# 0Setsuna0/SoftbodyUnity

Hardware: AMD Instinct MI355X
Metric: particle-substeps/sec (higher is better)
Workload: dtype f32

## Files before the change

softbodyunity_amd/csrc/kernel_types.hpp:

```cpp
#pragma once
#include <hip/hip_runtime.h>
#include <stdint.h>

#include "stream_codec.hpp"

namespace sbk {

struct TickParams {
    float h, inv_h, hgx, hgy, hgz, kd, at_d, at_v, at_b;
    float pnx, pny, pnz, pd;
    int32_t plane_on;
    float pad[2];
};

constexpr int kKindFirst = 0, kKindMid = 1, kKindLast = 2, kKindLayer = 3, kKindPeek = 4, kKindMidKinematic = 5;
constexpr bool kind_is_kinematic(int k) { return k == kKindMidKinematic; }
constexpr int kind_base(int k) { return kind_is_kinematic(k) ? kKindMid : k; }
constexpr bool kind_has_mark(int k) { return k != kKindLayer; }
constexpr bool kind_rounds_before_mark(int k) { return k != kKindFirst; }
constexpr bool kind_rounds_after_mark(int k) { return k == kKindFirst || kind_base(k) == kKindMid; }
constexpr bool kind_ends_tick(int k) { return k == kKindLast || k == kKindPeek; }
constexpr bool kind_reads_prev(int k) { return kind_base(k) == kKindMid || k == kKindLast; }
constexpr bool kind_touches_prev(int k) { return k == kKindFirst || kind_reads_prev(k); }
constexpr bool kind_writes_peek(int k) { return k == kKindPeek; }
constexpr bool kind_may_read_ghosts(int k) { return k == kKindMid || k == kKindLast; }
constexpr bool kind_gathers(int k) { return k == kKindLayer; }

struct TileDesc {
    int32_t n_local, run_count, n_rounds;
    int32_t gather_begin;
    uint32_t s_begin;
    uint32_t s_hdr;
    uint32_t s_len;
    uint32_t packed_lanes;
    int32_t run_overflow;
    int32_t n_pal;
    int32_t n_steps;
    uint32_t s_items;
    int2 runs[10];
};
constexpr int kInlineRuns = 10;
constexpr int kWide8MaxTiles = 768;
#ifndef SB_REG_ROUNDS
#define SB_REG_ROUNDS 4
#endif
#ifndef SB_REG_ROUNDS_NARROW
#define SB_REG_ROUNDS_NARROW 3
#endif
constexpr int kRegRoundsWide = SB_REG_ROUNDS, kRegRoundsNarrow = SB_REG_ROUNDS_NARROW;
#ifdef SB_REG_COMPACT_ONLY
constexpr bool kRegFullSlots = false;
#else
constexpr bool kRegFullSlots = true;
#endif
constexpr bool kLanePackDecodable = kRegRoundsNarrow >= kLanePackRounds;
constexpr int kMaxRoundsLds = 128;

typedef float f32x3_t __attribute__((ext_vector_type(3)));
struct PosView {
    float *xyz;
    const float *w;
};

constexpr int kMaxMassPalette = 64;

struct TileArgs {
    PosView pos;
    const uint8_t *w8;
    const float *wpal;
    float *prev;
    float *vel;
    const TileDesc *tiles;
    const int2 *runs_overflow;
    const uint32_t *stream;
    const TickParams *tp;
    const int32_t *gather;
    int32_t max_local;
    int32_t rounds_dwords;
    int32_t pal_dwords;
    int32_t win_dwords;
    int32_t tile_base;
    int32_t w_uniform;
    int32_t item_waves;
    int32_t store_through;
    union {
        const float *ghost_src;
        uint2 *prev_code;
    };
    int32_t n_owned;
    float *peek_out;
    const int32_t *kin_map;
    float *kin_target;
};
constexpr int kHaloNone = 0, kHaloGhosts = 1;

constexpr int kNarrowTileThreads = 128;
constexpr int kQuadTileThreads = 512;
constexpr int kWideTileThreads = 256;
constexpr int kRoundSlots = 256;
constexpr int kSmallTile = 512, kLargeTile = 1024;
typedef float f32x3 __attribute__((ext_vector_type(3)));

typedef float f32x4 __attribute__((ext_vector_type(4)));
typedef uint32_t u32x4 __attribute__((ext_vector_type(4)));

constexpr int kMaxPeers = 8;
struct PeerSlot {
    int32_t n_send, n_recv;
    int32_t send_off[kMaxPeers + 1];
// ... 25 lines not shown
```

softbodyunity_amd/csrc/launch_shape.hpp:

```cpp
#pragma once
#include "kernel_types.hpp"
#include "tables_host.hpp"

namespace sbt {

struct LaunchShape { int threads, ppt; bool quads; };
inline bool same_width(const LaunchShape &a, const LaunchShape &b) { return a.threads == b.threads && a.ppt == b.ppt; }

constexpr LaunchShape kShapeNarrow{sbk::kNarrowTileThreads, sbk::kSmallTile / sbk::kNarrowTileThreads, false};
constexpr LaunchShape kShapeWide{sbk::kWideTileThreads, sbk::kSmallTile / sbk::kWideTileThreads, false};
constexpr LaunchShape kShapeWideLarge{sbk::kWideTileThreads, sbk::kLargeTile / sbk::kWideTileThreads, false};
constexpr LaunchShape kShapeEight{sbk::kQuadTileThreads, sbk::kSmallTile / sbk::kQuadTileThreads, false};
constexpr LaunchShape kShapeEightLarge{sbk::kQuadTileThreads, sbk::kLargeTile / sbk::kQuadTileThreads, false};

inline LaunchShape tile_launch_shape(const TilingScalars &D, int tile_lanes, int quad_lanes, int narrow_min_tiles, int n_tiles_in_launch, bool ghosts) {
    const bool small = D.max_local <= sbk::kSmallTile;
    const bool narrow = small && (D.packed_lanes ? D.packed_lanes == sbk::kLanePackLanes : (tile_lanes ? tile_lanes == sbk::kNarrowTileThreads : n_tiles_in_launch >= narrow_min_tiles));
    const bool quad8 = D.has_quads && quad_lanes == sbk::kQuadTileThreads;
    const bool wide8 = small && !D.has_quads && !D.packed_lanes && (tile_lanes ? tile_lanes == sbk::kQuadTileThreads : n_tiles_in_launch <= sbk::kWide8MaxTiles);
    const bool quads = ghosts ? false : D.has_quads;
    LaunchShape sh = quads && quad8 ? (small ? kShapeEight : kShapeEightLarge) : wide8 ? kShapeEight : narrow ? kShapeNarrow : small ? kShapeWide : kShapeWideLarge;
    sh.quads = quads;
    return sh;
}

inline bool tiling_always_narrow(const TilingScalars &D, int tile_lanes) {
    if (D.n_tiles == 0) return true;
    return D.max_local <= sbk::kSmallTile && !D.has_quads && (D.packed_lanes ? D.packed_lanes == sbk::kLanePackLanes : tile_lanes == sbk::kNarrowTileThreads);
}
constexpr int64_t kPrevCodeMaxParticles = (int64_t)1 << 26;
struct PrevCodeInputs {
    int world = 1;
    int halo_slots = 0;
    int tile_lanes = 0;
    bool w_palette = false;
    int steps_between_tiles = 0;
    int64_t n_local = 0;
};
inline bool use_prev_codes(const TilingScalars &T0, const TilingScalars &T1, const PrevCodeInputs &in) {
    if (in.world != 1 || in.halo_slots != 0) return false;
    if (!in.w_palette) return false;
    if (in.steps_between_tiles != 0) return false;
    if (T0.n_tiles == 0 || in.n_local > kPrevCodeMaxParticles) return false;
    return tiling_always_narrow(T0, in.tile_lanes) && tiling_always_narrow(T1, in.tile_lanes);
}

}
```

softbodyunity_amd/csrc/schedule.hip:

```cpp
#include "solver_internal.hpp"
#include "launch_shape.hpp"
#include "tile_kernel.hip.hpp"
#include "aux_kernels.hip.hpp"

namespace sbi {

sbk::TickParams tick_params(const sb_solver *s, float dt, int substeps) {
    sbk::TickParams t{};
    volatile float S = (float)substeps;
    volatile float h = dt / S;
    t.h = h;
    volatile float inv_h = 1.0f / h;
    t.inv_h = inv_h;
    volatile float hx = h * s->desc.gravity[0], hy = h * s->desc.gravity[1], hz = h * s->desc.gravity[2];
    t.hgx = hx; t.hgy = hy; t.hgz = hz;
    volatile float td = s->desc.damping * h;
    volatile float kd = 1.0f - td;
    t.kd = kd < 0.0f ? 0.0f : (float)kd;
    volatile float h2 = h * h;
    volatile float ad = s->mesh->kind[0].compliance / h2;
    volatile float av = s->mesh->kind[1].compliance / h2;
    volatile float av36 = 36.0f * av;
    volatile float ab = s->mesh->kind[2].compliance / h2;
    t.at_d = ad; t.at_v = av36; t.at_b = ab;
// ... 108 lines not shown

void halo_exchange_calls(sb_solver *s, int slot, hipStream_t st) {
    if (!halo_slot_active(s, slot) || s->peer.enabled) return;
    DevHalo &D = *s->halos[slot];
    const size_t fl = sbt::ghost_floats((size_t)slot);
    for (size_t k = 0; k < D.peers.size(); ++k) {
        int cs = D.send_off[k + 1] - D.send_off[k], cr = D.recv_off[k + 1] - D.recv_off[k];
        if (s->loopback) cs = cr = std::min(cs, cr);
        if (cs) NCCL_CHECK(rccl().Send(s->d_sendbuf.p + fl * D.send_off[k], fl * (size_t)cs, ncclFloat, s->loopback ? 0 : D.peers[k], s->comm, st));
        if (cr) NCCL_CHECK(rccl().Recv(s->d_recvbuf.p + fl * D.recv_off[k], fl * (size_t)cr, ncclFloat, s->loopback ? 0 : D.peers[k], s->comm, st));
    }
}

void halo_exchange_post(sb_solver *s, int slot, hipStream_t st) {
    if (!halo_slot_active(s, slot) || s->peer.enabled) return;
    launch_halo_unpack(s, *s->halos[slot], slot, st);
}

void ExchangeTimer::mark(hipStream_t st, bool join) {
    Event e;
    if (free_list.empty()) e.create(); else { e = std::move(free_list.back()); free_list.pop_back(); }
    HIP_CHECK(hipEventRecord(e, st));
    (join ? join_pending : pending).push_back(std::move(e));
}
void ExchangeTimer::recycle() {
    for (auto *v : {&pending, &join_pending}) {
        free_list.insert(free_list.end(), std::make_move_iterator(v->begin()), std::make_move_iterator(v->end()));
        v->clear();
    }
}

void halo_exchange(sb_solver *s, int slot, hipStream_t st) {
    if (!st) st = s->stream;
    if (!halo_slot_active(s, slot)) return;
    const bool timed = s->xtimer.enabled && !s->capturing;
    if (timed) s->xtimer.mark(st);
    if (!s->peer.enabled) halo_exchange_pre(s, slot, st);
    if (timed) s->xtimer.mark(st);
    if (s->peer.enabled) halo_exchange_pre(s, slot, st);
    if (!s->peer.enabled) {
        NCCL_CHECK(rccl().GroupStart());
        try {
            halo_exchange_calls(s, slot, st);
        } catch (...) {
            (void)rccl().GroupEnd();
            throw;
        }
        NCCL_CHECK(rccl().GroupEnd());
    }
    halo_exchange_post(s, slot, st);
    if (timed) s->xtimer.mark(st);
}

template <int KIND, bool Q, int THREADS, int PPT, bool W, int G, bool C = false>
void launch_tile_kernel(const sb_solver *s, const DevTiling &D, const sbk::TileDesc *tiles_at_base, int n_wg, const sbk::TileArgs &A) {
    hipLaunchKernelGGL((sbk::tile_kernel<KIND, Q, THREADS, PPT, W, G, C>), dim3(n_wg), dim3(THREADS), D.lds_bytes + s->lds_pad, s->stream, tiles_at_base, n_wg, A);
}
template <int KIND, bool Q, bool W, int G>
void launch_tile_shaped(const sb_solver *s, const DevTiling &D, const sbt::LaunchShape &sh, const sbk::TileDesc *tiles_at_base, int n_wg, const sbk::TileArgs &A) {
    using namespace sbt;
    if (same_width(sh, kShapeEight)) return launch_tile_kernel<KIND, Q, kShapeEight.threads, kShapeEight.ppt, W, G>(s, D, tiles_at_base, n_wg, A);
    if constexpr (Q) if (same_width(sh, kShapeEightLarge)) return launch_tile_kernel<KIND, Q, kShapeEightLarge.threads, kShapeEightLarge.ppt, W, G>(s, D, tiles_at_base, n_wg, A);
    if (same_width(sh, kShapeNarrow)) return launch_tile_kernel<KIND, Q, kShapeNarrow.threads, kShapeNarrow.ppt, W, G>(s, D, tiles_at_base, n_wg, A);
    if (same_width(sh, kShapeWide)) return launch_tile_kernel<KIND, Q, kShapeWide.threads, kShapeWide.ppt, W, G>(s, D, tiles_at_base, n_wg, A);
    if (same_width(sh, kShapeWideLarge)) return launch_tile_kernel<KIND, Q, kShapeWideLarge.threads, kShapeWideLarge.ppt, W, G>(s, D, tiles_at_base, n_wg, A);
    throw std::runtime_error("internal: no tile kernel is built for the launch shape asked for");
}

template <int KIND>
void launch_tile(sb_solver *s, DevTiling &D, int tile_begin = 0, int tile_end = -1, int halo = sbk::kHaloNone, const sbk::TileDesc *table = nullptr) {
    const bool ghosts = halo == sbk::kHaloGhosts;
    if (tile_end < 0) tile_end = D.n_tiles;
    if (tile_end <= tile_begin) return;
    sbk::TileArgs A{};
    A.pos = s->pos_view(); A.w8 = s->d_w8.p; A.wpal = s->d_wpal.p; A.prev = s->d_prev.p; A.vel = s->d_vel.p;
    A.tiles = D.tiles.p; A.runs_overflow = D.runs_overflow.p; A.stream = D.stream.p;
    A.tp = s->d_tp.p;
    A.gather = D.gather.p;
    A.w_uniform = s->w_uniform ? 1 : 0;
    A.item_waves = D.item_waves;
    A.store_through = tile_end - tile_begin <= s->store_through_max_tiles ? 3 : s->store_through_large;
    A.ghost_src = ghosts ? s->d_recvbuf.p : nullptr; A.n_owned = (int32_t)s->n_owned;
    A.peek_out = sbk::kind_writes_peek(KIND) ? s->d_peek.p : nullptr;
    A.kin_map = sbk::kind_is_kinematic(KIND) ? s->d_kin_map.p : nullptr; A.kin_target = sbk::kind_is_kinematic(KIND) ? s->d_kin_target.p : nullptr;
    A.max_local = D.max_local; A.win_dwords = D.win_dwords; A.tile_base = tile_begin; A.pal_dwords = D.pal_dwords; A.rounds_dwords = D.rounds_dwords;
    const sbk::TileDesc *tiles_at_base = table ? table : D.tiles.p + tile_begin;
    const int n_wg = tile_end - tile_begin;
    const sbt::LaunchShape sh = sbt::tile_launch_shape(D, s->tile_lanes, s->quad_lanes, s->narrow_min_tiles, n_wg, ghosts);
    constexpr bool kCanGhost = sbk::kind_may_read_ghosts(KIND);
    if (ghosts && !(kCanGhost && !D.has_quads)) throw std::runtime_error("internal: ghost-reading tile kernel requested for a launch that has none");
    const bool W = s->w_palette;
    if constexpr (sbk::kind_touches_prev(KIND)) if (s->prev_codes) {
        if (ghosts || sh.quads || !W || !sbt::same_width(sh, sbt::kShapeNarrow)) throw std::runtime_error("internal: previous-position codes are on, but the launch is not 128 x 4 spring-only with palette masses");
        A.prev_code = s->d_prev_code.p;
        return launch_tile_kernel<KIND, false, sbt::kShapeNarrow.threads, sbt::kShapeNarrow.ppt, true, sbk::kHaloNone, true>(s, D, tiles_at_base, n_wg, A);
    }
    if (ghosts) {
        if constexpr (kCanGhost) W ? launch_tile_shaped<KIND, false, true, sbk::kHaloGhosts>(s, D, sh, tiles_at_base, n_wg, A) : launch_tile_shaped<KIND, false, false, sbk::kHaloGhosts>(s, D, sh, tiles_at_base, n_wg, A);
    } else if (sh.quads) W ? launch_tile_shaped<KIND, true, true, sbk::kHaloNone>(s, D, sh, tiles_at_base, n_wg, A) : launch_tile_shaped<KIND, true, false, sbk::kHaloNone>(s, D, sh, tiles_at_base, n_wg, A);
    else W ? launch_tile_shaped<KIND, false, true, sbk::kHaloNone>(s, D, sh, tiles_at_base, n_wg, A) : launch_tile_shaped<KIND, false, false, sbk::kHaloNone>(s, D, sh, tiles_at_base, n_wg, A);
}

struct LaunchTimer {
    std::vector<Event> ev;
    std::vector<int> slot;
    hipStream_t stream;
    void begin(int which) {
        Event a, b;
        a.create(); b.create();
        HIP_CHECK(hipEventRecord(a, stream));
        ev.push_back(std::move(a)); ev.push_back(std::move(b)); slot.push_back(which);
    }
    void end() { HIP_CHECK(hipEventRecord(ev.back(), stream)); }
};

void launch_tick_kernel(sb_solver *s, int it, int substeps, LaunchTimer *lt, int tile_begin = 0, int tile_end = -1, bool kin = false) {
    const int tl = s->plan->plan.tiling ? (it & 1) : 0;
    DevTiling &D = s->tiling[tl];
    if (lt && D.n_tiles) lt->begin(it == 0 ? 2 + (int)s->gcolours.size() : (it == substeps ? 3 + (int)s->gcolours.size() : tl));
    const int halo_in = s->fused_unpack && tl == 1 ? sbk::kHaloGhosts : sbk::kHaloNone;
    if (it == 0) launch_tile<sbk::kKindFirst>(s, D, tile_begin, tile_end);
    else if (it < substeps && kin) launch_tile<sbk::kKindMidKinematic>(s, D, tile_begin, tile_end);
    else if (it < substeps) launch_tile<sbk::kKindMid>(s, D, tile_begin, tile_end, halo_in);
    else launch_tile<sbk::kKindLast>(s, D, tile_begin, tile_end, halo_in);
    if (lt && D.n_tiles) lt->end();
}

void launch_t2_layer(sb_solver *s, int layer, LaunchTimer *lt, bool with_halo = true) {
    const auto rg = s->t2_layer_range[layer];
    if (with_halo) halo_exchange(s, 2 + (int)s->gcolours.size() + layer);
    if (rg.second <= rg.first) return;
    if (lt) lt->begin(4 + (int)s->gcolours.size());
    launch_tile<sbk::kKindLayer>(s, s->tiling[2], rg.first, rg.second);
    if (lt) lt->end();
}

void launch_gcolour(sb_solver *s, int gc, LaunchTimer *lt) {
    DevGColour &G = *s->gcolours[gc];
    if (G.count == 0) return;
    if (lt) lt->begin(2 + gc);
    dim3 grid((G.count + 255) / 256);
    if (G.type == 0)
        hipLaunchKernelGGL(sbk::global_distance_kernel, grid, dim3(256), 0, s->stream, s->pos_view(), G.ij.p, G.rest.p, G.count,
                           s->d_tp.p);
    else
        hipLaunchKernelGGL(sbk::global_quad_kernel, grid, dim3(256), 0, s->stream, s->pos_view(), G.quad.p, G.rest2.p, G.count,
                           G.type, s->d_tp.p);
// ... 416 lines not shown
```

softbodyunity_amd/csrc/solver_internal.hpp:

```cpp
#pragma once
#include <hip/hip_runtime.h>
#include <rccl/rccl.h>
#include <dlfcn.h>

#include <algorithm>
#include <array>
#include <atomic>
#include <chrono>
#include <climits>
#include <cmath>
#include <cstdio>
#include <cstdlib>
#include <cstring>
#include <limits>
#include <map>
#include <memory>
#include <mutex>
#include <type_traits>
#include <stdexcept>
#include <string>
#include <utility>
#include <vector>

#include "../../include/softbody.h"
// ... 95 lines not shown
    StepKind kind;
    TileRange range;
    bool kin;
    int it, substeps;
    int index;
};
struct TickShape { int substeps; bool fuse, defer_last, kin; };

struct ExchangeTimer {
    bool enabled = false;
    std::vector<Event> pending, join_pending, free_list;
    void mark(hipStream_t st, bool join = false);
    void recycle();
};

}

using sbi::DevBuf; using sbi::DevGColour; using sbi::DevHalo; using sbi::DevTiling;

struct sb_plan {
    sbp::Plan plan;
    sbp::LocalPlan local;
    bool owns_local = true;
};

struct sb_solver {
    sb_desc desc;
    bool finalized = false;
    sbi::Stream stream;
    sbi::Event ev0, ev1;
    ncclComm_t comm = nullptr;
    bool loopback = false;
    int schedule = SB_SCHEDULE_SERIAL_EAGER;
    uint64_t plan_hash = 0;
    sbi::Stream comm_stream;
    sbi::Event ev_boundary, ev_halo;
    bool overlap_halo = false;
    std::shared_ptr<sbi::AuthoredMesh> mesh = std::make_shared<sbi::AuthoredMesh>();
    bool sharded = false;
    sb_domain domain{};
    std::vector<int32_t> global_id;
    std::unique_ptr<sb_plan> plan;
    int64_t dev_bytes = 0;
    int64_t n_owned = 0, n_local = 0;
    DevBuf<float> d_pos3;
    DevBuf<float> d_wf;
    DevBuf<uint8_t> d_w8;
    DevBuf<float> d_wpal;
    bool w_palette = false;
    bool w_uniform = false;
    sbk::PosView pos_view() const { return sbk::PosView{d_pos3.p, d_wf.p}; }
    DevBuf<float> d_prev, d_vel;
    bool prev_codes = false;
    DevBuf<uint2> d_prev_code;
    DevBuf<sbk::TickParams> d_tp;
    DevBuf<float> d_sendbuf, d_recvbuf;
    DevTiling tiling[3];
    std::vector<std::pair<int32_t, int32_t>> t2_layer_range;
    std::vector<std::unique_ptr<DevGColour>> gcolours;
    std::vector<std::unique_ptr<DevHalo>> halos;
    sbk::TickParams tp_host{};
    bool tp_valid = false;
    sbi::GraphCache graphs;
    bool deferred = false;
    int deferred_substeps = 0;
    uint32_t tune_flags = 0;
    int win_dwords_cap = 0;
    int prev_offset_bytes = 0;
    bool lazy_tick = true;
    int tile_lanes = 0;
    int quad_lanes = 512;
    int store_through_max_tiles = 6144;
    int store_through_large = 0;
    int narrow_min_tiles = 10240;
    size_t lds_pad = 0;
    bool pack_tiles = true;
    bool fused_unpack = false;
    bool graph_rccl = false;
    std::vector<float> h_stage;
    struct AutoSchedule {
        int state = 0;
        int tick = 0;
        sbi::Event ev[8];
        int n[2] = {0, 0};
        double decided_ms[2] = {0, 0};
    } calib;
    bool group_walk = false;
    bool capturing = false;
    sbi::ExchangeTimer xtimer;
    struct PeerState {
        bool enabled = false, linked = false, fine_grained = false;
        uint32_t *mailbox = nullptr;
        size_t bytes = 0, data_off_words = 0, off_table = 0;
        int n_slots = 0;
        std::vector<uint32_t *> remote;
        std::vector<uint8_t> opened;
        std::vector<std::vector<uint32_t>> my_off;
        std::vector<sbk::PeerSlot> slots;
        DevBuf<uint32_t> local;
        sbi::HostBuf<uint32_t> h_error;
        size_t slot_base(int slot, int world) const { return sbt::mailbox_slot_base(slot, world); }
        ~PeerState() {
            for (size_t r = 0; r < remote.size(); ++r) if (opened[r] && remote[r]) (void)hipIpcCloseMemHandle(remote[r]);
            if (mailbox) (void)hipFree(mailbox);
        }
    } peer;
// ... 121 lines not shown
```

softbodyunity_amd/csrc/tables.hip:

```cpp
#include "solver_internal.hpp"
#include "launch_shape.hpp"

namespace sbi {

sbp::Input make_input(const float *rest, int32_t n, const int32_t *d, int64_t md, const int32_t *v, int64_t mv,
                      const int32_t *b, int64_t mb) {
    sbp::Input in;
    in.rest = rest; in.n = n; in.dist_ij = d; in.m_d = md; in.vol = v; in.m_v = mv; in.bend = b; in.m_b = mb;
    return in;
}

sbp::Domain to_domain(const sb_domain &d) {
    sbp::Domain D;
    D.set = true; D.n_global = d.n_global; D.ell = d.spacing; D.fill = d.fill > 0 && d.fill <= 1 ? d.fill : 1.0;
    for (int a = 0; a < 3; ++a) { D.lo[a] = d.lo[a]; D.hi[a] = d.hi[a]; }
    return D;
}
sbp::Opts plan_opts(int rank, int world, const int32_t dims[3], int32_t tile_particles, int32_t partition, uint32_t plan_flags,
                    int64_t m_v, int64_t m_b, const sb_domain *domain) {
    sbp::Opts o;
    if (domain) {
        o.domain = to_domain(*domain);
        if (domain->four_vertex_constraints) m_v += 1;
    }
// ... 71 lines not shown
    opt.peer_enabled = s->peer.enabled; opt.sharded = s->sharded; opt.plan_hash = s->plan_hash;
    opt.plan_shape = opt.peer_enabled && L.world > 1 ? plan_shape(s) : 0u;
    sbt::HostTables H;
    sbt::build_state(in, opt, H);
    s->n_owned = H.n_owned; s->n_local = H.n_local;
    s->w_palette = H.w_palette; s->w_uniform = H.w_uniform;
    s->d_pos3.upload(H.pos3, s->dev_bytes);
    s->d_wf.upload(H.wf, s->dev_bytes);
    if (H.w_palette) s->d_w8.upload(H.w8, s->dev_bytes);
    s->d_wpal.upload(H.wpal, s->dev_bytes);
    s->d_vel.upload(H.vel, s->dev_bytes);
    for (std::vector<float> *v : {&H.pos3, &H.wf, &H.vel}) std::vector<float>().swap(*v);
    std::vector<uint8_t>().swap(H.w8);
    s->d_prev.alloc((size_t)s->n_local * 3, s->dev_bytes, (size_t)s->prev_offset_bytes / sizeof(float));
    HIP_CHECK(hipMemset(s->d_prev.p, 0, (size_t)s->n_local * 3 * sizeof(float)));
    s->d_tp.alloc(1, s->dev_bytes);
    for (int tl = 0; tl < 3; ++tl) {
        sbt::build_tiling(in, opt, tl, H);
        sbt::HostTiling &T = H.T[tl];
        DevTiling &D = s->tiling[tl];
        static_cast<sbt::TilingScalars &>(D) = T;
        D.tiles.upload(T.tiles, s->dev_bytes); D.runs_overflow.upload(T.runs_overflow, s->dev_bytes);
        D.stream.upload(T.stream, s->dev_bytes);
        D.gather.upload(T.gather, s->dev_bytes);
        T.release_arrays();
    }
    s->t2_layer_range = H.t2_layer_range;
    sbt::build_gcolours(in, H);
    for (const sbt::HostGColour &G : H.gcolours) {
        auto D = std::make_unique<DevGColour>();
        D->type = G.type; D->count = G.count;
        if (G.type == 0) { D->ij.upload(G.ij, s->dev_bytes); D->rest.upload(G.rest, s->dev_bytes); }
        else { D->quad.upload(G.quad, s->dev_bytes); D->rest2.upload(G.rest2, s->dev_bytes); }
        s->gcolours.push_back(std::move(D));
    }
    sbt::build_halos(in, opt, H);
    for (sbt::HostHalo &G : H.halos) {
        auto D = std::make_unique<DevHalo>();
        D->send_idx.upload(G.send_idx, s->dev_bytes); D->recv_idx.upload(G.recv_idx, s->dev_bytes);
        D->peers = std::move(G.peers); D->send_off = std::move(G.send_off); D->recv_off = std::move(G.recv_off);
        s->halos.push_back(std::move(D));
    }
    s->d_sendbuf.alloc(H.send_floats, s->dev_bytes);
    s->d_recvbuf.alloc(H.recv_floats, s->dev_bytes);
    if (H.recv_floats) HIP_CHECK(hipMemset(s->d_recvbuf.p, 0, H.recv_floats * sizeof(float)));
    s->fused_unpack = H.fused_unpack;
    if (s->peer.enabled && L.world > 1) alloc_mailbox(s, H.mailbox);
    sbt::PrevCodeInputs pc;
    pc.world = s->desc.world; pc.tile_lanes = s->tile_lanes; pc.w_palette = s->w_palette; pc.n_local = s->n_local;
    pc.halo_slots = s->loopback ? 1 : 0;
    for (const auto &D : s->halos) if (D->active()) ++pc.halo_slots;
    pc.steps_between_tiles = (int)s->t2_layer_range.size() + (int)s->gcolours.size();
    s->prev_codes = sbt::use_prev_codes(s->tiling[0], s->tiling[1], pc);
    if (s->prev_codes) {
        s->d_prev_code.alloc((size_t)s->n_local, s->dev_bytes);
        HIP_CHECK(hipMemset(s->d_prev_code.p, 0, (size_t)s->n_local * sizeof(uint2)));
    }
}

}
```

softbodyunity_amd/csrc/tile_kernel.hip.hpp:

```cpp
#pragma once
#include "device_math.hip.hpp"
#include "prev_code.hpp"

namespace sbk {

__device__ __forceinline__ void lds_barrier() { asm volatile("s_waitcnt lgkmcnt(0)\n\ts_barrier" ::: "memory"); }

__device__ __forceinline__ void decode_compact_distance(uint32_t e, const float *s_pal, int &i, int &k, float &L0) { i = compact_slot_i(e); k = compact_slot_j(e); L0 = s_pal[compact_slot_pal(e)]; }
__device__ __forceinline__ void decode_full_distance(const uint2 e, int &i, int &k, float &L0) { i = pair_i(e.x); k = pair_j(e.x); L0 = __uint_as_float(e.y); }
__device__ __forceinline__ void read_distance_slot(const uint32_t *slots, int c, bool compact, const float *s_pal, int &i, int &k, float &L0) {
    if (compact) decode_compact_distance(slots[c], s_pal, i, k, L0);
    else decode_full_distance(*reinterpret_cast<const uint2 *>(slots + kFullSlotDwords * c), i, k, L0);
}

__device__ __forceinline__ void quad_slot_offsets(const uint4 &e, int q, int &o0, int &o1, int &o2, int &o3) {
    o0 = 4 * (int)pair_i(e.x) + q; o1 = 4 * (int)pair_j(e.x) + q;
    o2 = 4 * (int)pair_i(e.y) + q; o3 = 4 * (int)pair_j(e.y) + q;
}

template <bool QUADS, int THREADS> constexpr int kWavesPerSimd = QUADS ? (THREADS == 64 ? 3 : (THREADS == 512 ? 2 : 4)) : (THREADS == 256 ? 8 : (THREADS == 128 ? 6 : 4));
template <int KIND_, bool QUADS, int THREADS, int PPT, bool WPAL, int HALO = kHaloNone, bool CODED = false>
__global__ __launch_bounds__(THREADS, (kWavesPerSimd<QUADS, THREADS> - (KIND_ == 5 && !QUADS ? 1 : 0))) void tile_kernel(const TileDesc *tiles_at_base, int n_workgroups, TileArgs A) {
    constexpr int KIND = kind_base(KIND_);
    constexpr bool KIN = kind_is_kinematic(KIND_);
    constexpr bool GHOSTS = HALO == kHaloGhosts;
    constexpr int kTileThreads = THREADS;
    constexpr int kCPL = THREADS >= kRoundSlots ? 1 : kRoundSlots / THREADS;
    extern __shared__ uint4 lds_raw[];
    float4 *lds_pos = reinterpret_cast<float4 *>(lds_raw);
    uint32_t *s_rounds = reinterpret_cast<uint32_t *>(lds_pos + A.max_local);
    float *s_pal = reinterpret_cast<float *>(s_rounds + A.rounds_dwords);
    uint32_t *cbuf = s_rounds + A.rounds_dwords + A.pal_dwords;
    f32x3 *lds_spare = reinterpret_cast<f32x3 *>(cbuf + A.win_dwords);
    typedef const TileDesc __attribute__((address_space(4))) *ConstTileDescPtr;
#ifndef SB_NO_XCD_REMAP
    const int nwg = n_workgroups, wg = (int)blockIdx.x;
    const int xq = nwg >> 3, xr = nwg & 7, xcd = wg & 7;
    const int tile_index = (xcd < xr ? xcd * (xq + 1) : xr * (xq + 1) + (xcd - xr) * xq) + (wg >> 3);
#else
    const int tile_index = (int)blockIdx.x;
#endif
    const TileDesc __attribute__((address_space(4))) &td = *((ConstTileDescPtr)(uintptr_t)tiles_at_base + tile_index);
    const int n_rounds_all = td.n_rounds;
    const int tid = threadIdx.x;
    const int n_local = td.n_local;
    const int run_count = td.run_count;
    const TickParams tp = *A.tp;
    const uint32_t *tstream = A.stream + td.s_begin;
#if defined(SB_ABLATE) && SB_ABLATE == 4
    if (n_local >= 0) { if (n_rounds_all == 0x7fffffff) A.vel[0] = tp.h; return; }
#endif

    int g[PPT];
    if (kind_gathers(KIND_)) {
#pragma unroll
        for (int m = 0; m < PPT; ++m) {
            const int l = tid + m * kTileThreads;
            g[m] = l < n_local ? A.gather[td.gather_begin + l] : -1;
        }
    } else {
        int run_d[kInlineRuns], run_y[kInlineRuns];
#pragma unroll
        for (int r = 0; r < kInlineRuns; ++r) { run_y[r] = td.runs[r].y; run_d[r] = td.runs[r].x - td.runs[r].y; }
#pragma unroll
        for (int m = 0; m < PPT; ++m) {
            const int l = tid + m * kTileThreads;
            int d = run_d[0];
#pragma unroll
            for (int r = 1; r < kInlineRuns; ++r) d = l >= run_y[r] ? run_d[r] : d;
            int gi = l + d;
            if (run_count > kInlineRuns)
                for (int r = kInlineRuns; r < run_count; ++r) {
                    const int2 rn = A.runs_overflow[td.run_overflow + r - kInlineRuns];
                    if (rn.y <= l) gi = rn.x + (l - rn.y);
                }
            g[m] = l < n_local ? gi : -1;
        }
    }
    const int R = n_rounds_all;
    const int v_begin = kind_rounds_before_mark(KIND_) ? 0 : R;
    const int v_end = !kind_has_mark(KIND_) ? R : (kind_rounds_after_mark(KIND_) ? 2 * R + 1 : R + 1);
    const uint32_t d_lo = td.s_hdr;
    const uint32_t d_hi = td.s_len;
    const uint32_t win = (uint32_t)A.win_dwords;
    uint32_t win_lo = d_lo;
    auto load_window = [&](uint32_t lo) {
        const uint32_t n4 = (min(lo + win, d_hi) - lo) >> 2;
        const uint4 *src = reinterpret_cast<const uint4 *>(tstream + lo);
        uint4 *dst = reinterpret_cast<uint4 *>(cbuf);
        uint32_t t0 = (uint32_t)tid;
        asm volatile("" : "+v"(t0));
        for (uint32_t i = t0; i < n4; i += 4 * kTileThreads) {
            uint4 v0 = src[i], v1, v2, v3;
            const bool b1 = i + kTileThreads < n4, b2 = i + 2 * kTileThreads < n4, b3 = i + 3 * kTileThreads < n4;
            if (b1) v1 = src[i + kTileThreads];
            if (b2) v2 = src[i + 2 * kTileThreads];
            if (b3) v3 = src[i + 3 * kTileThreads];
            dst[i] = v0;
            if (b1) dst[i + kTileThreads] = v1;
            if (b2) dst[i + 2 * kTileThreads] = v2;
            if (b3) dst[i + 3 * kTileThreads] = v3;
        }
    };
    f32x4 X[PPT];
    float pvx[PPT], pvy[PPT], pvz[PPT];
    uint32_t wi[PPT];
    uint32_t pc_lo[PPT], pc_hi[PPT];
    const int mypal = WPAL ? __float_as_int(A.wpal[tid & (kMaxMassPalette - 1)]) : 0;
#pragma unroll
    for (int m = 0; m < PPT; ++m) {
        const int gc = max(g[m], 0);
        const bool ghost = GHOSTS && gc >= A.n_owned;
        const float *px = ghost ? A.ghost_src + 6 * (size_t)(gc - A.n_owned) : A.pos.xyz + 3 * (size_t)gc;
        X[m].x = px[0]; X[m].y = px[1]; X[m].z = px[2];
        if (WPAL) { wi[m] = A.w8[A.w_uniform ? 0 : gc]; X[m].w = 0.0f; } else { wi[m] = 0; X[m].w = A.pos.w[gc]; }
        pvx[m] = pvy[m] = pvz[m] = 0.0f;
        pc_lo[m] = pc_hi[m] = 0u;
        if (kind_reads_prev(KIND_)) {
            if (CODED) { const uint2 c = A.prev_code[gc]; pc_lo[m] = c.x; pc_hi[m] = c.y; }
            else {
                const float *pp = ghost ? px + 3 : A.prev + 3 * (size_t)gc;
                pvx[m] = pp[0]; pvy[m] = pp[1]; pvz[m] = pp[2];
            }
        }
    }
    const bool rounds_in_lds = n_rounds_all <= A.rounds_dwords;
    const uint32_t rw = tstream[max(min(tid, n_rounds_all - 1), 0)];
    const bool rounds_in_lanes = n_rounds_all <= 64;
    const uint32_t rwl = tstream[max(min(tid & 63, n_rounds_all - 1), 0)];
    uint32_t itreg = 0;
    if (QUADS && kTileThreads == 64 * A.item_waves) {
        const int ns = td.n_steps;
        itreg = tstream[ns > 0 ? td.s_items + (uint32_t)((tid >> 6) * ns + min(tid & 63, ns - 1)) : 0u];
    }
    const int n_pal = td.n_pal;
    const uint32_t palw = tstream[tid < n_pal ? ((n_rounds_all + 3) & ~3) + tid : 0];
#ifndef SB_KW
#define SB_KW (QUADS ? 4 : 2)
#endif
    constexpr int kW = SB_KW;
    const bool lane_packed = !QUADS && kTileThreads == kLanePackLanes && td.packed_lanes == (uint32_t)kLanePackLanes;
    const bool lane_packed_full = !WPAL && lane_packed && td.n_pal == 0;
    const bool wide_packed = !QUADS && kTileThreads == kWidePackLanes && td.packed_lanes == (uint32_t)kWidePackLanes;
    const bool any_packed = lane_packed || wide_packed;
    const uint32_t n4_first = wide_packed ? 0u : lane_packed ? (lane_packed_full ? 2u * (uint32_t)kLanePackLanes : (uint32_t)kLanePackLanes)
                                          : (min(win_lo + win, d_hi) - win_lo) >> 2;
    const u32x4 *wsrc = reinterpret_cast<const u32x4 *>(tstream + win_lo);
    u32x4 wv[kW];
#pragma unroll
    for (int q = 0; q < kW; ++q) {
        const uint32_t i = tid + q * kTileThreads;
        wv[q] = i < n4_first ? wsrc[i] : *reinterpret_cast<const u32x4 *>(tstream);
    }
    typedef uint32_t u32x2 __attribute__((ext_vector_type(2)));
    u32x2 wc = {0u, 0u};
    u32x2 wp = {0u, 0u};
    if (!QUADS && kTileThreads == kWidePackLanes)
        wp = *reinterpret_cast<const u32x2 *>(wide_packed ? tstream + win_lo + 2u * (uint32_t)tid : tstream);
#pragma unroll
    for (int m = 0; m < PPT; ++m) {
        if (CODED) asm volatile("" ::"v"(X[m].x), "v"(pc_lo[m]), "v"(wi[m]), "v"(X[m].w));
        else asm volatile("" ::"v"(X[m].x), "v"(pvx[m]), "v"(wi[m]), "v"(X[m].w));
    }
    asm volatile("" ::"v"(mypal));
    if (CODED && kind_reads_prev(KIND_)) {
        bool esc = false;
#pragma unroll
        for (int m = 0; m < PPT; ++m) {
            const Bits3 p = prev_decode((uint64_t)pc_lo[m] | ((uint64_t)pc_hi[m] << 32), Bits3{__float_as_uint(X[m].x), __float_as_uint(X[m].y), __float_as_uint(X[m].z)});
            pvx[m] = __uint_as_float(p.x); pvy[m] = __uint_as_float(p.y); pvz[m] = __uint_as_float(p.z);
            esc = esc || (g[m] >= 0 && prev_hi_is_escape(pc_hi[m]));
        }
        if (__builtin_amdgcn_ballot_w64(esc) != 0ull) {
#pragma unroll
            for (int m = 0; m < PPT; ++m)
                if (g[m] >= 0 && prev_hi_is_escape(pc_hi[m])) {
                    const float *pp = A.prev + 3 * (size_t)g[m];
                    pvx[m] = pp[0]; pvy[m] = pp[1]; pvz[m] = pp[2];
                }
        }
    }
    if (WPAL) {
#pragma unroll
        for (int m = 0; m < PPT; ++m) X[m].w = __int_as_float(__builtin_amdgcn_ds_bpermute((int)(wi[m] << 2), mypal));
    }
#pragma unroll
    for (int q = 0; q < kW; ++q) asm volatile("" ::"v"(wv[q].x));
    asm volatile("" ::"v"(rw), "v"(palw), "v"(rwl), "v"(itreg));
    if (!QUADS && kTileThreads == kWidePackLanes) asm volatile("" ::"v"(wp.x));
#pragma unroll
    for (int m = 0; m < PPT; ++m)
        if (g[m] >= 0) *reinterpret_cast<f32x4 *>(lds_pos + tid + m * kTileThreads) = X[m];
    if (rounds_in_lds && tid < n_rounds_all) s_rounds[tid] = rw;
    if (tid < n_pal) s_pal[tid] = __uint_as_float(palw);
    if (kTileThreads < kMaxRoundsLds && rounds_in_lds)
        for (int q = tid + kTileThreads; q < n_rounds_all; q += kTileThreads) s_rounds[q] = tstream[q];
    if (kTileThreads < kMaxPalette)
        for (int q = tid + kTileThreads; q < n_pal; q += kTileThreads) s_pal[q] = __uint_as_float(tstream[((n_rounds_all + 3) & ~3) + q]);
    {
        u32x4 *dst = reinterpret_cast<u32x4 *>(cbuf);
#pragma unroll
        for (int q = 0; q < kW; ++q) {
            const uint32_t i = tid + q * kTileThreads;
            if (i < n4_first && !any_packed) dst[i] = wv[q];
        }
        if (!any_packed)
            for (uint32_t i = tid + kW * kTileThreads; i < n4_first; i += kTileThreads) dst[i] = wsrc[i];
    }
    __syncthreads();
    if (!WPAL && !QUADS && kTileThreads == kLanePackLanes && lane_packed_full)
        wc = *reinterpret_cast<const u32x2 *>(tstream + win_lo + 8u * (uint32_t)kLanePackLanes + 2u * (uint32_t)tid);
#if defined(SB_ABLATE) && SB_ABLATE == 5
    if (n_local >= 0) { if (lds_pos[tid].x == 1.2345e-30f && cbuf[tid] == 0x12345678u) A.vel[0] = tp.h; return; }
#endif

    auto mark_step = [&]() {
#pragma unroll
        for (int m = 0; m < PPT; ++m)
            if (g[m] >= 0) {
                const int l = tid + m * kTileThreads;
                float4 P = lds_pos[l];
                if (KIND != kKindFirst && tp.plane_on && P.w > 0.0f) {
                    float a = tp.pnx * P.x, b = tp.pny * P.y, c = tp.pnz * P.z;
                    float pen = ((a + b) + c) - tp.pd;
                    if (pen < 0.0f) {
                        float dx = pen * tp.pnx, dy = pen * tp.pny, dz = pen * tp.pnz;
                        P.x = P.x - dx; P.y = P.y - dy; P.z = P.z - dz;
                        if (kind_ends_tick(KIND_)) lds_pos[l] = P;
                    }
                }
                if (KIND == kKindPeek) continue;
                float vx, vy, vz;
                const size_t o = 3 * (size_t)g[m];
                if (KIND == kKindFirst) {
                    vx = A.vel[o + 0]; vy = A.vel[o + 1]; vz = A.vel[o + 2];
                } else {
                    float dx = P.x - pvx[m], dy = P.y - pvy[m], dz = P.z - pvz[m];
                    float qx = dx * tp.inv_h, qy = dy * tp.inv_h, qz = dz * tp.inv_h;
                    vx = qx * tp.kd; vy = qy * tp.kd; vz = qz * tp.kd;
                }
                bool moved = false;
                if (KIN && P.w == 0.0f) {
                    const int ks = A.kin_map[g[m]];
                    if (ks >= 0) {
                        float *t = A.kin_target + 3 * (size_t)ks;
                        const float tx = t[0], ty = t[1], tz = t[2];
                        if (tx == tx) { P.x = tx; P.y = ty; P.z = tz; moved = true; t[0] = __int_as_float(0x7fc00000); }
                    }
                }
                if (KIND == kKindLast) {
                    A.vel[o + 0] = vx; A.vel[o + 1] = vy; A.vel[o + 2] = vz;
                } else {
                    if (CODED) { pvx[m] = P.x; pvy[m] = P.y; pvz[m] = P.z; }
                    else if (A.store_through & 1) store3_through(A.prev + o, P.x, P.y, P.z);
                    else { A.prev[o + 0] = P.x; A.prev[o + 1] = P.y; A.prev[o + 2] = P.z; }
                    if (P.w > 0.0f) {
                        vx = vx + tp.hgx; vy = vy + tp.hgy; vz = vz + tp.hgz;
                        float hx = tp.h * vx, hy = tp.h * vy, hz = tp.h * vz;
                        P.x = P.x + hx; P.y = P.y + hy; P.z = P.z + hz;
                        lds_pos[l] = P;
                    } else if (KIN && moved) lds_pos[l] = P;
                }
            }
    };

    constexpr int kRegRounds = THREADS >= 256 ? kRegRoundsWide : kRegRoundsNarrow;
    if (kRegRounds > 0 && !QUADS && n_rounds_all <= kRegRounds && n_rounds_all > 0 && (kRegFullSlots || n_pal > 0) && (any_packed || d_hi - d_lo <= win)) {
        const bool tile_compact = n_pal > 0;
        uint32_t rs[kRegRounds > 0 ? kRegRounds : 1][kCPL];
        float rl[kRegRounds > 0 ? kRegRounds : 1][kCPL];
        int rcnt[kRegRounds > 0 ? kRegRounds : 1];
        {
            uint32_t o = 0;
#pragma unroll
            for (int r = 0; r < kRegRounds; ++r) {
                rcnt[r] = 0;
                if (r < n_rounds_all) {
                    rcnt[r] = (int)group_dist_count((uint32_t)__builtin_amdgcn_readlane((int)rwl, r));
                    if (kCPL == 2 && lane_packed) {
#pragma unroll
                        for (int u = 0; u < kCPL; ++u) {
                            const int bit = kLanePackFieldBits * (2 * r + u), w0 = bit >> 5, sh = bit & 31;
                            const uint32_t lo = wv[0][w0] >> sh;
                            const uint32_t hi = (sh + kLanePackFieldBits > 32) ? (wv[0][w0 + 1 < kLaneWordDwords ? w0 + 1 : kLaneWordDwords - 1] << ((32 - sh) & 31)) : 0u;
                            const uint32_t f = (lo | hi) & kLanePackFieldMask;
                            rs[r][u] = compact_slot_of_pack_field(f);
                            if (!WPAL) {
                                const int fld = 2 * r + u;
                                rl[r][u] = __uint_as_float(fld < 4 ? wv[1][fld < 4 ? fld : 0] : wc[fld >= 4 ? fld - 4 : 0]);
                            }
                        }
                    } else if (kCPL == 1 && wide_packed) {
                        rs[r][0] = compact_slot_of_pack_field(wide_word_field(wp.x, wp.y, r < kLanePackRounds ? r : 0));
                    } else if (tile_compact) {
#pragma unroll
                        for (int u = 0; u < kCPL; ++u) {
                            const int c = tid + u * kTileThreads;
                            rs[r][u] = cbuf[o + (c < rcnt[r] ? c : 0)];
                        }
                        o += compact_data_dwords((uint32_t)rcnt[r]);
                    } else {
#pragma unroll
                        for (int u = 0; u < kCPL; ++u) {
                            const int c = tid + u * kTileThreads;
                            const uint2 e = *reinterpret_cast<const uint2 *>(cbuf + o + 2 * (c < rcnt[r] ? c : 0));
                            rs[r][u] = compact_slot_of_pair(e.x);
                            rl[r][u] = __uint_as_float(e.y);
                        }
                        o += full_data_dwords((uint32_t)rcnt[r]);
                    }
                } else {
#pragma unroll
                    for (int u = 0; u < kCPL; ++u) { rs[r][u] = 0; rl[r][u] = 0.0f; }
                }
            }
            if (tile_compact) {
#pragma unroll
                for (int r = 0; r < kRegRounds; ++r)
#pragma unroll
                    for (int u = 0; u < kCPL; ++u) rl[r][u] = s_pal[compact_slot_pal(rs[r][u])];
            }
        }
        auto reg_round = [&](const uint32_t (&e)[kCPL], const float (&L0)[kCPL], int cnt) {
            if (kCPL == 1) {
                if (tid < cnt) {
                    const int i = compact_slot_i(e[0]), k = compact_slot_j(e[0]);
                    float4 a = lds_pos[i], b = lds_pos[k];
                    if (project_distance(a, b, L0[0], tp.at_d)) { lds_pos[i] = a; lds_pos[k] = b; }
                }
            } else {
                int ci[kCPL], ck[kCPL];
                bool con[kCPL];
                f32x4 ca[kCPL], cb[kCPL];
#pragma unroll
                for (int u = 0; u < kCPL; ++u) {
                    con[u] = tid + u * kTileThreads < cnt;
                    ci[u] = compact_slot_i(e[u]); ck[u] = compact_slot_j(e[u]);
                    ca[u] = *reinterpret_cast<const f32x4 *>(lds_pos + ci[u]);
                    cb[u] = *reinterpret_cast<const f32x4 *>(lds_pos + ck[u]);
                }
#pragma unroll
                for (int u = 0; u < kCPL; ++u) {
                    float4 a = make_float4(ca[u].x, ca[u].y, ca[u].z, ca[u].w), b = make_float4(cb[u].x, cb[u].y, cb[u].z, cb[u].w);
                    con[u] = project_distance_nobranch(a, b, L0[u], tp.at_d) && con[u];
                    ca[u].x = a.x; ca[u].y = a.y; ca[u].z = a.z; cb[u].x = b.x; cb[u].y = b.y; cb[u].z = b.z;
                }
#pragma unroll
                for (int u = 0; u < kCPL; ++u) {
                    f32x3 *da = con[u] ? reinterpret_cast<f32x3 *>(lds_pos + ci[u]) : lds_spare;
                    f32x3 *db = con[u] ? reinterpret_cast<f32x3 *>(lds_pos + ck[u]) : lds_spare;
                    *da = (f32x3){ca[u].x, ca[u].y, ca[u].z};
                    *db = (f32x3){cb[u].x, cb[u].y, cb[u].z};
                }
            }
            lds_barrier();
        };
#if defined(SB_ABLATE) && SB_ABLATE == 1
        constexpr bool kRunRounds = false;
#else
        constexpr bool kRunRounds = true;
#endif
        if (kind_rounds_before_mark(KIND_) && kRunRounds) {
#pragma unroll
            for (int r = 0; r < kRegRounds; ++r) if (r < n_rounds_all) reg_round(rs[r], rl[r], rcnt[r]);
        }
        if (kind_has_mark(KIND_)) { mark_step(); lds_barrier(); }
        if (kind_rounds_after_mark(KIND_) && kRunRounds) {
#pragma unroll
            for (int r = 0; r < kRegRounds; ++r) if (r < n_rounds_all) reg_round(rs[r], rl[r], rcnt[r]);
        }
    } else if (QUADS && kTileThreads == 64 * A.item_waves && td.n_steps > 0 && d_hi - d_lo <= win) {
        const int n_steps = td.n_steps;
        const int wave = __builtin_amdgcn_readfirstlane(tid >> 6), lane = tid & 63;
        const uint32_t *items = tstream + td.s_items + (uint32_t)(wave * n_steps);
        float *lds_f = reinterpret_cast<float *>(lds_pos);
        const int q = tid & 3;
        auto run_pass = [&]() {
            if (n_steps > 64) itreg = items[min(lane, n_steps - 1)];
#if defined(SB_ABLATE) && SB_ABLATE == 1
            if (n_steps >= 0) return;
#endif
#pragma unroll 1
            for (int st = 0; st < n_steps; ++st) {
                if ((st & 63) == 0 && st > 0) itreg = items[min(st + lane, n_steps - 1)];
                const uint32_t it = (uint32_t)__builtin_amdgcn_readlane((int)itreg, st & 63);
                const uint32_t type = item_type(it);
                const int cnt = (int)item_count(it);
                const uint32_t *slots = cbuf + item_offset(it);
                if (type == kItemBending) {
                    const int c = lane >> 4;
                    if (c < cnt) {
                        const uint4 e = *reinterpret_cast<const uint4 *>(slots + 4 * c);
                        const int k = (lane >> 2) & 3;
                        int o0, o1, o2, o3;
                        quad_slot_offsets(e, q, o0, o1, o2, o3);
                        const float P[4] = {lds_f[o0], lds_f[o1], lds_f[o2], lds_f[o3]};
// ... 190 lines not shown
```

Measured before the change: 123.4 billion.

## Add lean coded tile kernel variant with uniform-mass and reduced LDS footprint

Adds a specialized 'lean' template variant of the tile kernel, used when every tile is lane-packed with register-resident rounds and prev codes are on. It drops LDS staging of rounds and of palette tails, shrinks the LDS allocation, cuts the window load width to one vector, and forces the register-rounds path. When all masses are uniform, it skips the per-particle mass load and bpermute and substitutes a launch-wide constant weight. The aim is to reduce LDS use, register pressure and global loads to raise occupancy, at the cost of more template instantiations and strict eligibility conditions.

New measurement: 130.6 billion (median of 6 runs). +5.8%, better.

```diff
diff --git a/softbodyunity_amd/csrc/kernel_types.hpp b/softbodyunity_amd/csrc/kernel_types.hpp
--- a/softbodyunity_amd/csrc/kernel_types.hpp
+++ b/softbodyunity_amd/csrc/kernel_types.hpp
@@ -55,6 +55,12 @@
 #endif
 constexpr bool kLanePackDecodable = kRegRoundsNarrow >= kLanePackRounds;
 constexpr int kMaxRoundsLds = 128;
+constexpr int kLeanOff = 0, kLeanPalette = 1, kLeanUniform = 2;
+#ifdef SB_LEAN_NO_UNIFORM
+constexpr bool kLeanUniformMass = false;
+#else
+constexpr bool kLeanUniformMass = true;
+#endif
 
 typedef float f32x3_t __attribute__((ext_vector_type(3)));
 struct PosView {
diff --git a/softbodyunity_amd/csrc/launch_shape.hpp b/softbodyunity_amd/csrc/launch_shape.hpp
--- a/softbodyunity_amd/csrc/launch_shape.hpp
+++ b/softbodyunity_amd/csrc/launch_shape.hpp
@@ -45,4 +45,15 @@
     return tiling_always_narrow(T0, in.tile_lanes) && tiling_always_narrow(T1, in.tile_lanes);
 }
 
+inline bool tiling_all_lane_packed(const TilingScalars &D) {
+    if (D.n_tiles == 0) return true;
+    return D.packed_lanes == sbk::kLanePackLanes && D.n_packed_tiles == (int64_t)D.n_tiles &&
+           D.rounds_dwords <= ((sbk::kRegRoundsNarrow + 3) & ~3);
 }
+inline bool use_lean_coded(const TilingScalars &T0, const TilingScalars &T1, const PrevCodeInputs &in) {
+    if (!use_prev_codes(T0, T1, in) || !sbk::kLanePackDecodable) return false;
+    return tiling_all_lane_packed(T0) && tiling_all_lane_packed(T1);
+}
+inline size_t lean_lds_bytes(const TilingScalars &D) { return (size_t)D.max_local * sizeof(float4) + (size_t)D.pal_dwords * 4 + 16; }
+
+}
diff --git a/softbodyunity_amd/csrc/schedule.hip b/softbodyunity_amd/csrc/schedule.hip
--- a/softbodyunity_amd/csrc/schedule.hip
+++ b/softbodyunity_amd/csrc/schedule.hip
@@ -184,9 +184,10 @@
     if (timed) s->xtimer.mark(st);
 }
 
-template <int KIND, bool Q, int THREADS, int PPT, bool W, int G, bool C = false>
+template <int KIND, bool Q, int THREADS, int PPT, bool W, int G, bool C = false, int LEAN = sbk::kLeanOff>
 void launch_tile_kernel(const sb_solver *s, const DevTiling &D, const sbk::TileDesc *tiles_at_base, int n_wg, const sbk::TileArgs &A) {
-    hipLaunchKernelGGL((sbk::tile_kernel<KIND, Q, THREADS, PPT, W, G, C>), dim3(n_wg), dim3(THREADS), D.lds_bytes + s->lds_pad, s->stream, tiles_at_base, n_wg, A);
+    const size_t lds = LEAN != sbk::kLeanOff ? sbt::lean_lds_bytes(D) : D.lds_bytes;
+    hipLaunchKernelGGL((sbk::tile_kernel<KIND, Q, THREADS, PPT, W, G, C, LEAN>), dim3(n_wg), dim3(THREADS), lds + s->lds_pad, s->stream, tiles_at_base, n_wg, A);
 }
 template <int KIND, bool Q, bool W, int G>
 void launch_tile_shaped(const sb_solver *s, const DevTiling &D, const sbt::LaunchShape &sh, const sbk::TileDesc *tiles_at_base, int n_wg, const sbk::TileArgs &A) {
@@ -225,6 +226,11 @@
     if constexpr (sbk::kind_touches_prev(KIND)) if (s->prev_codes) {
         if (ghosts || sh.quads || !W || !sbt::same_width(sh, sbt::kShapeNarrow)) throw std::runtime_error("internal: previous-position codes are on, but the launch is not 128 x 4 spring-only with palette masses");
         A.prev_code = s->d_prev_code.p;
+        if (s->lean_coded) {
+            constexpr sbt::LaunchShape N = sbt::kShapeNarrow;
+            if constexpr (!sbk::kind_is_kinematic(KIND)) if (s->w_uniform && sbk::kLeanUniformMass) return launch_tile_kernel<KIND, false, N.threads, N.ppt, true, sbk::kHaloNone, true, sbk::kLeanUniform>(s, D, tiles_at_base, n_wg, A);
+            return launch_tile_kernel<KIND, false, N.threads, N.ppt, true, sbk::kHaloNone, true, sbk::kLeanPalette>(s, D, tiles_at_base, n_wg, A);
+        }
         return launch_tile_kernel<KIND, false, sbt::kShapeNarrow.threads, sbt::kShapeNarrow.ppt, true, sbk::kHaloNone, true>(s, D, tiles_at_base, n_wg, A);
     }
     if (ghosts) {
diff --git a/softbodyunity_amd/csrc/solver_internal.hpp b/softbodyunity_amd/csrc/solver_internal.hpp
--- a/softbodyunity_amd/csrc/solver_internal.hpp
+++ b/softbodyunity_amd/csrc/solver_internal.hpp
@@ -171,6 +171,7 @@
     sbk::PosView pos_view() const { return sbk::PosView{d_pos3.p, d_wf.p}; }
     DevBuf<float> d_prev, d_vel;
     bool prev_codes = false;
+    bool lean_coded = false;
     DevBuf<uint2> d_prev_code;
     DevBuf<sbk::TickParams> d_tp;
     DevBuf<float> d_sendbuf, d_recvbuf;
diff --git a/softbodyunity_amd/csrc/tables.hip b/softbodyunity_amd/csrc/tables.hip
--- a/softbodyunity_amd/csrc/tables.hip
+++ b/softbodyunity_amd/csrc/tables.hip
@@ -147,6 +147,7 @@
     for (const auto &D : s->halos) if (D->active()) ++pc.halo_slots;
     pc.steps_between_tiles = (int)s->t2_layer_range.size() + (int)s->gcolours.size();
     s->prev_codes = sbt::use_prev_codes(s->tiling[0], s->tiling[1], pc);
+    s->lean_coded = sbt::use_lean_coded(s->tiling[0], s->tiling[1], pc);
     if (s->prev_codes) {
         s->d_prev_code.alloc((size_t)s->n_local, s->dev_bytes);
         HIP_CHECK(hipMemset(s->d_prev_code.p, 0, (size_t)s->n_local * sizeof(uint2)));
diff --git a/softbodyunity_amd/csrc/tile_kernel.hip.hpp b/softbodyunity_amd/csrc/tile_kernel.hip.hpp
--- a/softbodyunity_amd/csrc/tile_kernel.hip.hpp
+++ b/softbodyunity_amd/csrc/tile_kernel.hip.hpp
@@ -19,8 +19,10 @@
 }
 
 template <bool QUADS, int THREADS> constexpr int kWavesPerSimd = QUADS ? (THREADS == 64 ? 3 : (THREADS == 512 ? 2 : 4)) : (THREADS == 256 ? 8 : (THREADS == 128 ? 6 : 4));
-template <int KIND_, bool QUADS, int THREADS, int PPT, bool WPAL, int HALO = kHaloNone, bool CODED = false>
+template <int KIND_, bool QUADS, int THREADS, int PPT, bool WPAL, int HALO = kHaloNone, bool CODED = false, int LEAN = kLeanOff>
 __global__ __launch_bounds__(THREADS, (kWavesPerSimd<QUADS, THREADS> - (KIND_ == 5 && !QUADS ? 1 : 0))) void tile_kernel(const TileDesc *tiles_at_base, int n_workgroups, TileArgs A) {
+    static_assert(LEAN == kLeanOff || (CODED && WPAL && !QUADS && THREADS == kLanePackLanes && HALO == kHaloNone && !kind_writes_peek(KIND_) && kind_touches_prev(KIND_)),
+                  "LEAN: coded 128-lane spring-only launches with palette masses, no ghosts, no peek");
     constexpr int KIND = kind_base(KIND_);
     constexpr bool KIN = kind_is_kinematic(KIND_);
     constexpr bool GHOSTS = HALO == kHaloGhosts;
@@ -29,9 +31,9 @@
     extern __shared__ uint4 lds_raw[];
     float4 *lds_pos = reinterpret_cast<float4 *>(lds_raw);
     uint32_t *s_rounds = reinterpret_cast<uint32_t *>(lds_pos + A.max_local);
-    float *s_pal = reinterpret_cast<float *>(s_rounds + A.rounds_dwords);
+    float *s_pal = reinterpret_cast<float *>(s_rounds + (LEAN ? 0 : A.rounds_dwords));
     uint32_t *cbuf = s_rounds + A.rounds_dwords + A.pal_dwords;
-    f32x3 *lds_spare = reinterpret_cast<f32x3 *>(cbuf + A.win_dwords);
+    f32x3 *lds_spare = reinterpret_cast<f32x3 *>(LEAN ? s_rounds + A.pal_dwords : cbuf + A.win_dwords);
     typedef const TileDesc __attribute__((address_space(4))) *ConstTileDescPtr;
 #ifndef SB_NO_XCD_REMAP
     const int nwg = n_workgroups, wg = (int)blockIdx.x;
@@ -106,14 +108,17 @@
     float pvx[PPT], pvy[PPT], pvz[PPT];
     uint32_t wi[PPT];
     uint32_t pc_lo[PPT], pc_hi[PPT];
-    const int mypal = WPAL ? __float_as_int(A.wpal[tid & (kMaxMassPalette - 1)]) : 0;
+    constexpr bool kUniformW = LEAN == kLeanUniform;
+    const int mypal = WPAL && !kUniformW ? __float_as_int(A.wpal[tid & (kMaxMassPalette - 1)]) : 0;
+    const float w_launch = kUniformW ? A.wpal[0] : 0.0f;
 #pragma unroll
     for (int m = 0; m < PPT; ++m) {
         const int gc = max(g[m], 0);
         const bool ghost = GHOSTS && gc >= A.n_owned;
         const float *px = ghost ? A.ghost_src + 6 * (size_t)(gc - A.n_owned) : A.pos.xyz + 3 * (size_t)gc;
         X[m].x = px[0]; X[m].y = px[1]; X[m].z = px[2];
-        if (WPAL) { wi[m] = A.w8[A.w_uniform ? 0 : gc]; X[m].w = 0.0f; } else { wi[m] = 0; X[m].w = A.pos.w[gc]; }
+        if (kUniformW) { wi[m] = 0; X[m].w = w_launch; }
+        else if (WPAL) { wi[m] = A.w8[A.w_uniform ? 0 : gc]; X[m].w = 0.0f; } else { wi[m] = 0; X[m].w = A.pos.w[gc]; }
         pvx[m] = pvy[m] = pvz[m] = 0.0f;
         pc_lo[m] = pc_hi[m] = 0u;
         if (kind_reads_prev(KIND_)) {
@@ -125,7 +130,7 @@
         }
     }
     const bool rounds_in_lds = n_rounds_all <= A.rounds_dwords;
-    const uint32_t rw = tstream[max(min(tid, n_rounds_all - 1), 0)];
+    const uint32_t rw = LEAN ? 0u : tstream[max(min(tid, n_rounds_all - 1), 0)];
     const bool rounds_in_lanes = n_rounds_all <= 64;
     const uint32_t rwl = tstream[max(min(tid & 63, n_rounds_all - 1), 0)];
     uint32_t itreg = 0;
@@ -138,15 +143,15 @@
 #ifndef SB_KW
 #define SB_KW (QUADS ? 4 : 2)
 #endif
-    constexpr int kW = SB_KW;
-    const bool lane_packed = !QUADS && kTileThreads == kLanePackLanes && td.packed_lanes == (uint32_t)kLanePackLanes;
+    constexpr int kW = LEAN ? 1 : SB_KW;
+    const bool lane_packed = LEAN ? true : !QUADS && kTileThreads == kLanePackLanes && td.packed_lanes == (uint32_t)kLanePackLanes;
     const bool lane_packed_full = !WPAL && lane_packed && td.n_pal == 0;
     const bool wide_packed = !QUADS && kTileThreads == kWidePackLanes && td.packed_lanes == (uint32_t)kWidePackLanes;
     const bool any_packed = lane_packed || wide_packed;
     const uint32_t n4_first = wide_packed ? 0u : lane_packed ? (lane_packed_full ? 2u * (uint32_t)kLanePackLanes : (uint32_t)kLanePackLanes)
                                           : (min(win_lo + win, d_hi) - win_lo) >> 2;
     const u32x4 *wsrc = reinterpret_cast<const u32x4 *>(tstream + win_lo);
-    u32x4 wv[kW];
+    u32x4 wv[kW < 2 ? 2 : kW];
 #pragma unroll
     for (int q = 0; q < kW; ++q) {
         const uint32_t i = tid + q * kTileThreads;
@@ -159,10 +164,11 @@
         wp = *reinterpret_cast<const u32x2 *>(wide_packed ? tstream + win_lo + 2u * (uint32_t)tid : tstream);
 #pragma unroll
     for (int m = 0; m < PPT; ++m) {
-        if (CODED) asm volatile("" ::"v"(X[m].x), "v"(pc_lo[m]), "v"(wi[m]), "v"(X[m].w));
+        if (kUniformW) asm volatile("" ::"v"(X[m].x), "v"(pc_lo[m]));
+        else if (CODED) asm volatile("" ::"v"(X[m].x), "v"(pc_lo[m]), "v"(wi[m]), "v"(X[m].w));
         else asm volatile("" ::"v"(X[m].x), "v"(pvx[m]), "v"(wi[m]), "v"(X[m].w));
     }
-    asm volatile("" ::"v"(mypal));
+    if (!kUniformW) asm volatile("" ::"v"(mypal));
     if (CODED && kind_reads_prev(KIND_)) {
         bool esc = false;
 #pragma unroll
@@ -180,22 +186,23 @@
                 }
         }
     }
-    if (WPAL) {
+    if (WPAL && !kUniformW) {
 #pragma unroll
         for (int m = 0; m < PPT; ++m) X[m].w = __int_as_float(__builtin_amdgcn_ds_bpermute((int)(wi[m] << 2), mypal));
     }
 #pragma unroll
     for (int q = 0; q < kW; ++q) asm volatile("" ::"v"(wv[q].x));
-    asm volatile("" ::"v"(rw), "v"(palw), "v"(rwl), "v"(itreg));
+    if (LEAN) asm volatile("" ::"v"(palw), "v"(rwl));
+    else asm volatile("" ::"v"(rw), "v"(palw), "v"(rwl), "v"(itreg));
     if (!QUADS && kTileThreads == kWidePackLanes) asm volatile("" ::"v"(wp.x));
 #pragma unroll
     for (int m = 0; m < PPT; ++m)
         if (g[m] >= 0) *reinterpret_cast<f32x4 *>(lds_pos + tid + m * kTileThreads) = X[m];
-    if (rounds_in_lds && tid < n_rounds_all) s_rounds[tid] = rw;
+    if (!LEAN && rounds_in_lds && tid < n_rounds_all) s_rounds[tid] = rw;
     if (tid < n_pal) s_pal[tid] = __uint_as_float(palw);
     if (kTileThreads < kMaxRoundsLds && rounds_in_lds)
         for (int q = tid + kTileThreads; q < n_rounds_all; q += kTileThreads) s_rounds[q] = tstream[q];
-    if (kTileThreads < kMaxPalette)
+    if (!LEAN && kTileThreads < kMaxPalette)
         for (int q = tid + kTileThreads; q < n_pal; q += kTileThreads) s_pal[q] = __uint_as_float(tstream[((n_rounds_all + 3) & ~3) + q]);
     {
         u32x4 *dst = reinterpret_cast<u32x4 *>(cbuf);
@@ -211,7 +218,7 @@
     if (!WPAL && !QUADS && kTileThreads == kLanePackLanes && lane_packed_full)
         wc = *reinterpret_cast<const u32x2 *>(tstream + win_lo + 8u * (uint32_t)kLanePackLanes + 2u * (uint32_t)tid);
 #if defined(SB_ABLATE) && SB_ABLATE == 5
-    if (n_local >= 0) { if (lds_pos[tid].x == 1.2345e-30f && cbuf[tid] == 0x12345678u) A.vel[0] = tp.h; return; }
+    if (n_local >= 0) { if (lds_pos[tid].x == 1.2345e-30f && (LEAN ? wv[0].x : cbuf[tid]) == 0x12345678u) A.vel[0] = tp.h; return; }
 #endif
 
     auto mark_step = [&]() {
@@ -220,6 +227,7 @@
             if (g[m] >= 0) {
                 const int l = tid + m * kTileThreads;
                 float4 P = lds_pos[l];
+                if constexpr (kUniformW) P.w = w_launch;
                 if (KIND != kKindFirst && tp.plane_on && P.w > 0.0f) {
                     float a = tp.pnx * P.x, b = tp.pny * P.y, c = tp.pnz * P.z;
                     float pen = ((a + b) + c) - tp.pd;
@@ -265,8 +273,8 @@
     };
 
     constexpr int kRegRounds = THREADS >= 256 ? kRegRoundsWide : kRegRoundsNarrow;
-    if (kRegRounds > 0 && !QUADS && n_rounds_all <= kRegRounds && n_rounds_all > 0 && (kRegFullSlots || n_pal > 0) && (any_packed || d_hi - d_lo <= win)) {
-        const bool tile_compact = n_pal > 0;
+    if (LEAN || (kRegRounds > 0 && !QUADS && n_rounds_all <= kRegRounds && n_rounds_all > 0 && (kRegFullSlots || n_pal > 0) && (any_packed || d_hi - d_lo <= win))) {
+        const bool tile_compact = LEAN ? true : n_pal > 0;
         uint32_t rs[kRegRounds > 0 ? kRegRounds : 1][kCPL];
         float rl[kRegRounds > 0 ? kRegRounds : 1][kCPL];
         int rcnt[kRegRounds > 0 ? kRegRounds : 1];
@@ -342,6 +350,7 @@
 #pragma unroll
                 for (int u = 0; u < kCPL; ++u) {
                     float4 a = make_float4(ca[u].x, ca[u].y, ca[u].z, ca[u].w), b = make_float4(cb[u].x, cb[u].y, cb[u].z, cb[u].w);
+                    if constexpr (kUniformW) { a.w = w_launch; b.w = w_launch; }
                     con[u] = project_distance_nobranch(a, b, L0[u], tp.at_d) && con[u];
                     ca[u].x = a.x; ca[u].y = a.y; ca[u].z = a.z; cb[u].x = b.x; cb[u].y = b.y; cb[u].z = b.z;
                 }
```
